# Starlight0798/gymRL

Measured on AMD Instinct MI355X. Metric: env-steps/sec at N envs/GPU (PPO LunarLander), 1/2/4/8 GPUs + %HBM roofline, higher is better.
Workload: dtype f32; 1 GPU; PPO LunarLander-v3, 4096 vectorised envs per MI355X (BASELINE.json configs[1]); envs_per_gpu=4096, rollout_len=2048, num_epochs=10, num_minibatches=32, minibatch=262144, model=ActorCritic 8-256-256-{256-4,256-1} tanh, 200,965 params, parallelism=single GPU

## Files before the change

### gymrl_amd/csrc/env_lunar_device.hpp

```cpp
#pragma once
#include "env_common.hpp"

namespace gymrl {
namespace lunar {


constexpr float kScale = 30.0f;
constexpr float kW = 600.0f / kScale;
constexpr float kH = 400.0f / kScale;
constexpr float kHelipadY = kH / 4.0f;
constexpr float kLegDown = 18.0f / kScale;
constexpr float kLegAway = 20.0f / kScale;
constexpr float kDt = 1.0f / 50.0f;
constexpr int kVelIters = 180, kPosIters = 60, kMaxSteps = 1000;
constexpr float kLinearSlopSqMax = 0x1.a36e30p-16f;
constexpr float kLinearSlop = 0.005f, kAngularSlop = 2.0f / 180.0f * 3.14159265359f;
constexpr float kPolyRadius = 2.0f * kLinearSlop;
constexpr float kMaxLinCorr = 0.2f, kMaxAngCorr = 8.0f / 180.0f * 3.14159265359f;
constexpr float kBaumgarte = 0.2f;
constexpr float kMaxTranslation = 2.0f, kMaxRotation = 0.5f * 3.14159265359f;
constexpr float kTimeToSleep = 0.5f, kLinSleepTol = 0.01f, kAngSleepTol = 2.0f / 180.0f * 3.14159265359f;
constexpr float kMotorTorque = 40.0f;

__device__ constexpr float kInvM[3] = {0.20761245674740486f, 14.0625f, 14.0625f};
// ... 294 lines not shown
    if (action == 2) {
      m_power = 1.0f;
      const float ox = tipx * (4.0f / kScale + 2.0f * disp0) + sidex * disp1;
      const float oy = -tipy * (4.0f / kScale + 2.0f * disp0) - sidey * disp1;
      const float ipx = posx + ox, ipy = posy + oy;
      const float Ix = -ox * 13.0f * m_power, Iy = -oy * 13.0f * m_power;
      B[0].vx += kInvM[0] * Ix; B[0].vy += kInvM[0] * Iy;
      B[0].w += kInvI[0] * cross2(ipx - B[0].cx, ipy - B[0].cy, Ix, Iy);
    }
    if (action == 1 || action == 3) {
      const float dir = (float)(action - 2);
      s_power = 1.0f;
      const float ox = tipx * disp0 + sidex * (3.0f * disp1 + dir * 12.0f / kScale);
      const float oy = -tipy * disp0 - sidey * (3.0f * disp1 + dir * 12.0f / kScale);
      const float ipx = posx + ox - tipx * 17.0f / kScale;
      const float ipy = posy + oy + tipy * 14.0f / kScale;
      const float Ix = -ox * 0.6f * s_power, Iy = -oy * 0.6f * s_power;
      B[0].vx += kInvM[0] * Ix; B[0].vy += kInvM[0] * Iy;
      B[0].w += kInvI[0] * cross2(ipx - B[0].cx, ipy - B[0].cy, Ix, Iy);
    }
  }

  uint32_t my_touch = 0u;
  bool my_contact = false;
  {
    const Body me = select_body(B, mb);
    float px, py, qs, qc;
    body_xf(me, lcy_, px, py, qs, qc);
    float minx = 3.4e38f, maxx = -3.4e38f, miny = 3.4e38f;
    if (is_hull) {
#pragma unroll
      for (int i = 0; i < 6; ++i) {
        const float x = (qc * kHullVx[i] - qs * kHullVy[i]) + px, y = (qs * kHullVx[i] + qc * kHullVy[i]) + py;
        minx = fminf(minx, x); maxx = fmaxf(maxx, x); miny = fminf(miny, y);
      }
    } else {
#pragma unroll
      for (int i = 0; i < 4; ++i) {
        const float x = (qc * kLegVx[i] - qs * kLegVy[i]) + px, y = (qs * kLegVx[i] + qc * kLegVy[i]) + py;
        minx = fminf(minx, x); maxx = fmaxf(maxx, x); miny = fminf(miny, y);
      }
    }
    int e_lo = (int)floorf((minx - 2.0f * kPolyRadius) * 0.5f);
    int e_hi = (int)floorf((maxx + 2.0f * kPolyRadius) * 0.5f);
    e_lo = e_lo < 0 ? 0 : e_lo;
    e_hi = e_hi > 9 ? 9 : e_hi;
    int ocount[2]; uint32_t okey[2][2]; float oni[2][2], oti[2][2];
#pragma unroll
    for (int os = 0; os < 2; ++os) {
      ocount[os] = (int)lds.mu(os, MF_COUNT);
#pragma unroll
      for (int q = 0; q < 2; ++q) {
        okey[os][q] = lds.mu(os, MF_P0 + 5 * q + P_KEY);
        oni[os][q] = lds.mf(os, MF_P0 + 5 * q + P_NI);
        oti[os][q] = lds.mf(os, MF_P0 + 5 * q + P_TI);
      }
    }
    const int old_e0 = W.edge0;
    W.edge0 = e_lo;
#pragma nounroll
    for (int s = 0; s < 2; ++s) {
      Manifold mf;
      mf.count = 0; mf.faceB = 0; mf.lnx = mf.lny = mf.lpx = mf.lpy = 0.0f;
      mf.p[0] = ContactPt{0.0f, 0.0f, 0u, 0.0f, 0.0f}; mf.p[1] = mf.p[0];
      const int e = e_lo + s;
      if (e <= e_hi && e >= 0 && e <= 9) {
        float y1 = W.ty[0], y2 = W.ty[1];
#pragma unroll
        for (int k = 0; k < 10; ++k) if (k == e) { y1 = W.ty[k]; y2 = W.ty[k + 1]; }
        const float x1 = 2.0f * (float)e, x2 = 2.0f * (float)(e + 1);
        if (miny - 2.0f * kPolyRadius <= fmaxf(y1, y2)) {
          const float ccx = is_hull ? me.cx : px, ccy = is_hull ? me.cy : py;
          if (is_hull) collide_edge_polygon<6>(mf, kHullVx, kHullVy, kHullNx, kHullNy, px, py, qs, qc, ccx, ccy, x1, y1, x2, y2);
          else collide_edge_polygon<4>(mf, kLegVx, kLegVy, kLegNx, kLegNy, px, py, qs, qc, ccx, ccy, x1, y1, x2, y2);
        }
#pragma unroll
        for (int k = 0; k < 2; ++k) {
          mf.p[k].ni = 0.0f; mf.p[k].ti = 0.0f;
          if (k < mf.count) {
            bool found = false;
#pragma unroll
            for (int os = 0; os < 2; ++os) {
              if (old_e0 + os == e) {
#pragma unroll
                for (int q = 0; q < 2; ++q)
                  if (!found && q < ocount[os] && okey[os][q] == mf.p[k].key) {
                    mf.p[k].ni = oni[os][q]; mf.p[k].ti = oti[os][q]; found = true;
                  }
              }
            }
          }
        }
        if (mf.count > 0) { my_touch |= 1u << e; my_contact = true; }
      }
      lds.mu(s, MF_COUNT) = (uint32_t)mf.count; lds.mu(s, MF_FACEB) = (uint32_t)mf.faceB;
      lds.mf(s, MF_LNX) = mf.lnx; lds.mf(s, MF_LNY) = mf.lny;
      lds.mf(s, MF_LPX) = mf.lpx; lds.mf(s, MF_LPY) = mf.lpy;
#pragma unroll
      for (int k = 0; k < 2; ++k) {
        lds.mf(s, MF_P0 + 5 * k + P_LPX) = mf.p[k].lpx; lds.mf(s, MF_P0 + 5 * k + P_LPY) = mf.p[k].lpy;
        lds.mu(s, MF_P0 + 5 * k + P_KEY) = mf.p[k].key;
        lds.mf(s, MF_P0 + 5 * k + P_NI) = mf.p[k].ni; lds.mf(s, MF_P0 + 5 * k + P_TI) = mf.p[k].ti;
      }
    }
  }
  const uint32_t touching_now = quad_bcast_u<0>(my_touch) | (quad_bcast_u<1>(my_touch) << 10) |
                                (quad_bcast_u<2>(my_touch) << 20);
  const bool any_contact = touching_now != 0u;
  {
    const uint32_t began = touching_now & ~W.touching, ended = W.touching & ~touching_now;
    if (began & 0x3FFu) W.flags |= 4u;
#pragma unroll
    for (int L = 0; L < 2; ++L) {
#pragma unroll
      for (int e = 0; e < 10; ++e) {
        const uint32_t bit = 1u << (10 * (L + 1) + e);
        if (began & bit) W.flags |= (1u << L);
        if (ended & bit) W.flags &= ~(1u << L);
      }
    }
    W.touching = touching_now;
  }

  LUNAR_PROF_MARK(pt1);
  LUNAR_PROF_ADD(lds, 0, pt0, pt1);
  const float h = kDt;
#pragma unroll
  for (int b = 0; b < 3; ++b) {
    const float Fx = b == 0 ? fx : 0.0f, Fy = b == 0 ? fy : 0.0f;
    B[b].vx += h * (0.0f + kInvM[b] * Fx);
    B[b].vy += h * (-10.0f + kInvM[b] * Fy);
  }

  int vcn[2] = {0, 0};
  float vcf[2][16], vim[2][4];
#pragma unroll
  for (int s = 0; s < 2; ++s) {
#pragma unroll
    for (int f = 0; f < 16; ++f) vcf[s][f] = 0.0f;
    vim[s][0] = vim[s][1] = vim[s][2] = vim[s][3] = 0.0f;
  }
  if (any_contact) {
    Body me = select_body(B, mb);
    if (my_contact) {
      float px, py, qs, qc;
      body_xf(me, lcy_, px, py, qs, qc);
#pragma unroll
      for (int s = 0; s < 2; ++s) {
        const int count = (int)lds.mu(s, MF_COUNT);
        int vcount = count;
        if (count > 0) {
          const bool faceB = lds.mu(s, MF_FACEB) != 0u;
          const float lnx = lds.mf(s, MF_LNX), lny = lds.mf(s, MF_LNY);
          const float lpx = lds.mf(s, MF_LPX), lpy = lds.mf(s, MF_LPY);
          float nx, ny, wpx[2], wpy[2];
          if (!faceB) {
            nx = lnx; ny = lny;
#pragma unroll
            for (int k = 0; k < 2; ++k) {
              const float qx = lds.mf(s, MF_P0 + 5 * k + P_LPX), qy = lds.mf(s, MF_P0 + 5 * k + P_LPY);
              const float clx = (qc * qx - qs * qy) + px, cly = (qs * qx + qc * qy) + py;
              const float d = kPolyRadius - dot2(clx - lpx, cly - lpy, nx, ny);
              const float cAx = clx + d * nx, cAy = cly + d * ny;
              const float cBx = clx - kPolyRadius * nx, cBy = cly - kPolyRadius * ny;
              wpx[k] = 0.5f * (cAx + cBx); wpy[k] = 0.5f * (cAy + cBy);
            }
          } else {
            nx = qc * lnx - qs * lny; ny = qs * lnx + qc * lny;
            const float ppx = (qc * lpx - qs * lpy) + px, ppy = (qs * lpx + qc * lpy) + py;
#pragma unroll
            for (int k = 0; k < 2; ++k) {
              const float clx = lds.mf(s, MF_P0 + 5 * k + P_LPX), cly = lds.mf(s, MF_P0 + 5 * k + P_LPY);
              const float d = kPolyRadius - dot2(clx - ppx, cly - ppy, nx, ny);
              const float cBx = clx + d * nx, cBy = cly + d * ny;
              const float cAx = clx - kPolyRadius * nx, cAy = cly - kPolyRadius * ny;
              wpx[k] = 0.5f * (cAx + cBx); wpy[k] = 0.5f * (cAy + cBy);
            }
            nx = -nx; ny = -ny;
          }
          const float tx = ny, ty = -nx;
          float rx[2], ry[2];
#pragma unroll
          for (int k = 0; k < 2; ++k) {
            rx[k] = wpx[k] - me.cx; ry[k] = wpy[k] - me.cy;
            const float rn = cross2(rx[k], ry[k], nx, ny);
            const float kn = mB_ + iB_ * rn * rn;
            vcf[s][VC_NM0 - 1 + k] = kn > 0.0f ? 1.0f / kn : 0.0f;
            const float rt = cross2(rx[k], ry[k], tx, ty);
            const float kt = mB_ + iB_ * rt * rt;
            vcf[s][VC_TM0 - 1 + k] = kt > 0.0f ? 1.0f / kt : 0.0f;
            vcf[s][VC_RX0 - 1 + 2 * k] = rx[k]; vcf[s][VC_RY0 - 1 + 2 * k] = ry[k];
          }
          vcf[s][VC_NX - 1] = nx; vcf[s][VC_NY - 1] = ny;
          if (count == 2) {
            const float rn1 = cross2(rx[0], ry[0], nx, ny), rn2 = cross2(rx[1], ry[1], nx, ny);
            const float k11 = mB_ + iB_ * rn1 * rn1, k22 = mB_ + iB_ * rn2 * rn2, k12 = mB_ + iB_ * rn1 * rn2;
            if (k11 * k11 < 1000.0f * (k11 * k22 - k12 * k12)) {
              float det = k11 * k22 - k12 * k12;
              if (det != 0.0f) det = 1.0f / det;
              vcf[s][VC_K11 - 1] = k11; vcf[s][VC_K12 - 1] = k12; vcf[s][VC_K22 - 1] = k22;
              vcf[s][VC_I11 - 1] = det * k22; vcf[s][VC_I12 - 1] = -det * k12; vcf[s][VC_I22 - 1] = det * k11;
            } else {
              vcount = 1;
            }
          }
          vim[s][0] = lds.mf(s, MF_P0 + P_NI); vim[s][1] = lds.mf(s, MF_P0 + P_TI);
          vim[s][2] = lds.mf(s, MF_P1 + P_NI); vim[s][3] = lds.mf(s, MF_P1 + P_TI);
#pragma unroll
          for (int k = 0; k < 2; ++k) {
            if (k < vcount) {
              const float ni = vim[s][2 * k], ti = vim[s][2 * k + 1];
              const float Px = ni * nx + ti * tx, Py = ni * ny + ti * ty;
              me.w += iB_ * cross2(rx[k], ry[k], Px, Py);
              me.vx += mB_ * Px; me.vy += mB_ * Py;
            }
          }
        }
        vcn[s] = vcount;
      }
    }
    quad_share_velocity(B, me);
  }

  float jrAx[2], jrAy[2], jrBx[2], jrBy[2];
  float K11[2], K12[2], K13[2], K22[2], K23[2], K33[2], mmass[2];
  {
    float qsA, qcA;
    det_sincosf(B[0].a, &qsA, &qcA);
#pragma unroll
    for (int jj = 0; jj < 2; ++jj) {
      const int L = 1 - jj;
      const int bi = L + 1;
      float qsB, qcB;
      det_sincosf(B[bi].a, &qsB, &qcB);
      const float lax = 0.0f - 0.0f, lay = 0.0f - kHullLcY;
      const float lbx = leg_sign(L) * kLegAway, lby = kLegDown;
      jrAx[L] = qcA * lax - qsA * lay; jrAy[L] = qsA * lax + qcA * lay;
      jrBx[L] = qcB * lbx - qsB * lby; jrBy[L] = qsB * lbx + qcB * lby;
      const float mA = kInvM[0], mB = kInvM[bi], iA = kInvI[0], iB = kInvI[bi];
      K11[L] = mA + mB + jrAy[L] * jrAy[L] * iA + jrBy[L] * jrBy[L] * iB;
      K12[L] = -jrAy[L] * jrAx[L] * iA - jrBy[L] * jrBx[L] * iB;
      K13[L] = -jrAy[L] * iA - jrBy[L] * iB;
      K22[L] = mA + mB + jrAx[L] * jrAx[L] * iA + jrBx[L] * jrBx[L] * iB;
      K23[L] = jrAx[L] * iA + jrBx[L] * iB;
      K33[L] = iA + iB;
      mmass[L] = 1.0f / (iA + iB);
      Joint& J = W.j[L];
      const float ang = B[bi].a - B[0].a;
      if (ang <= joint_lower(L)) { if (J.state != 1) J.iz = 0.0f; J.state = 1; }
      else if (ang >= joint_upper(L)) { if (J.state != 2) J.iz = 0.0f; J.state = 2; }
      else { J.state = 0; J.iz = 0.0f; }
      const float Px = J.ix, Py = J.iy;
      B[0].vx -= mA * Px; B[0].vy -= mA * Py;
      B[0].w -= iA * (cross2(jrAx[L], jrAy[L], Px, Py) + J.im + J.iz);
      B[bi].vx += mB * Px; B[bi].vy += mB * Py;
      B[bi].w += iB * (cross2(jrBx[L], jrBy[L], Px, Py) + J.im + J.iz);
    }
  }

  LUNAR_PROF_MARK(pt2);
  LUNAR_PROF_ADD(lds, 1, pt1, pt2);
  float jpAx[2], jpAy[2], jpBx[2], jpBy[2];
  float c1x[2], c1y[2], c1z[2], det3i[2], det2i[2], lim_sign[2];
  bool at_limit[2];
#pragma unroll
  for (int L = 0; L < 2; ++L) {
    const float a11 = K11[L], a12 = K12[L], a13 = K13[L], a22 = K22[L], a23 = K23[L], a33 = K33[L];
    c1x[L] = a22 * a33 - a23 * a23; c1y[L] = a23 * a13 - a12 * a33; c1z[L] = a12 * a23 - a22 * a13;
    float det = a11 * c1x[L] + a12 * c1y[L] + a13 * c1z[L];
    if (det != 0.0f) det = 1.0f / det;
    det3i[L] = det;
    float d2 = a11 * a22 - a12 * a12;
    if (d2 != 0.0f) d2 = 1.0f / d2;
    det2i[L] = d2;
    jpAx[L] = -jrAy[L]; jpAy[L] = jrAx[L]; jpBx[L] = -jrBy[L]; jpBy[L] = jrBx[L];
    at_limit[L] = W.j[L].state != 0;
    lim_sign[L] = W.j[L].state == 1 ? 1.0f : -1.0f;
  }
  const bool r0 = role == 0, r1 = role == 1, r2 = role == 2;
  auto lane3 = [&](float x, float y, float z) { return r0 ? x : (r1 ? y : (r2 ? z : 0.0f)); };
  float JPA[2], JPB[2], C1[2], P2[2], Q2[2], A2[2], P3[2], Q3[2], A3[2], A3C[2], D2[2], MBv[2], IBz[2];
#pragma unroll
  for (int L = 0; L < 2; ++L) {
    const float a11 = K11[L], a12 = K12[L], a13 = K13[L], a22 = K22[L], a23 = K23[L], a33 = K33[L];
    JPA[L] = lane3(jpAx[L], jpAy[L], 0.0f); JPB[L] = lane3(jpBx[L], jpBy[L], 0.0f);
    C1[L] = lane3(c1x[L], c1y[L], c1z[L]);
    P2[L] = lane3(a23, a33, a13); Q2[L] = lane3(a13, a23, a33); A2[L] = lane3(a13, a11, a12);
    P3[L] = lane3(a23, a12, a22); Q3[L] = lane3(a12, a22, a23); A3[L] = lane3(a12, a13, a11);
    A3C[L] = lane3(a13, a23, 0.0f); D2[L] = lane3(a22, a11, 0.0f);
    MBv[L] = lane3(kInvM[L + 1], kInvM[L + 1], kInvI[L + 1]); IBz[L] = r2 ? kInvI[L + 1] : 0.0f;
  }
  const float MAv = lane3(kInvM[0], kInvM[0], kInvI[0]), IAz = r2 ? kInvI[0] : 0.0f;
  float VA = lane3(B[0].vx, B[0].vy, B[0].w);
  float VB[2] = {lane3(B[1].vx, B[1].vy, B[1].w), lane3(B[2].vx, B[2].vy, B[2].w)};
  float JI[2] = {lane3(W.j[0].ix, W.j[0].iy, W.j[0].iz), lane3(W.j[1].ix, W.j[1].iy, W.j[1].iz)};
  float IM[2] = {W.j[0].im, W.j[1].im};
  const float maxImp = h * kMotorTorque;
#define SB __builtin_amdgcn_sched_barrier(0)
#define USEL(c, a, b) (__builtin_unpredictable(c) ? (a) : (b))
  float zb[2];
  zb[1] = quad_perm<0xAA>(JI[1]) * A3C[1];
  zb[0] = 0.0f;
  float lim_nan[2] = {at_limit[0] ? lim_sign[0] : __builtin_nanf(""), at_limit[1] ? lim_sign[1] : __builtin_nanf("")};
  asm volatile("" : "+v"(lim_nan[0]), "+v"(lim_nan[1]));
  auto joints = [&]() {
#pragma unroll
    for (int jj = 0; jj < 2; ++jj) {
      const int L = 1 - jj;
      const bool lim = at_limit[L];
      float t = VB[L] - VA; SB;
      t = t - 0.3f * leg_sign(L); SB;
      float imp = -mmass[L] * t; SB;
      float nw = IM[L] + imp; SB;
      nw = __builtin_amdgcn_fmed3f(nw, -maxImp, maxImp); SB;
      imp = nw - IM[L]; IM[L] = nw; SB;
      const float mb_ = IBz[L] * imp; SB;
      VB[L] = VB[L] + mb_; SB;
      const float ma_ = IAz * imp; SB;
      VA = VA - ma_; SB;
      const float xb = quad_perm<0xAA>(VB[L]) * JPB[L]; SB;
      float c = VB[L] + xb; SB;
      const float xa = quad_perm<0xAA>(VA) * JPA[L]; SB;
      c = c - VA; SB;
      c = c - xa; SB;
      const float u1 = c * C1[L]; SB;
      const float zc = zb[L] - c; SB;
      const float q2 = quad_perm<kRot1>(c) * Q2[L]; SB;
      const float q3 = quad_perm<kRot2>(c) * Q3[L]; SB;
      const float m2 = c * P2[L] - q2; SB;
      const float m3 = c * P3[L] - q3; SB;
      float s1 = quad_perm<kRot1>(u1) + u1; SB;
      const float u2 = A2[L] * m2; SB;
      const float u3 = A3[L] * m3; SB;
      s1 = quad_perm<kRot2>(u1) + s1; SB;
      const float rr = USEL(lim, zc, -c); SB;
      float s2 = quad_perm<kRot1>(u2) + u2; SB;
      float s3 = quad_perm<kRot1>(u3) + u3; SB;
      const float d2r = D2[L] * rr; SB;
      s2 = quad_perm<kRot2>(u2) + s2; SB;
      s3 = quad_perm<kRot2>(u3) + s3; SB;
      const float r2_ = quad_perm<kSwap01>(rr) * K12[L]; SB;
      float sel = USEL(r1, s2, s3); SB;
      sel = USEL(r0, s1, sel); SB;
      const float nsol = -(det3i[L] * sel); SB;
      const float newJ = JI[L] + nsol; SB;
      const float uu = d2r - r2_; SB;
      const float u = det2i[L] * uu; SB;
      const float rt = quad_perm<0xAA>(newJ) * lim_nan[L]; SB;
      const float altz = USEL(lim, -JI[L], 0.0f); SB;
      const float alt = USEL(r2, altz, u); SB;
      float ip;
      asm("v_cmp_nge_f32 vcc, %1, 0\n\tv_cndmask_b32_e32 %0, %2, %3, vcc" : "=v"(ip) : "v"(rt), "v"(nsol), "v"(alt) : "vcc"); SB;
      JI[L] = JI[L] + ip; SB;
      zb[1 - L] = quad_perm<0xAA>(JI[1 - L]) * A3C[1 - L]; SB;
      const float ay = quad_perm<0x55>(ip) * jrAx[L]; SB;
      const float ax = quad_perm<0x00>(ip) * jrAy[L]; SB;
      const float by = quad_perm<0x55>(ip) * jrBx[L]; SB;
      const float bx = quad_perm<0x00>(ip) * jrBy[L]; SB;
      const float crA = ay - ax; SB;
      const float crB = by - bx; SB;
      const float wA = crA + ip; SB;
      const float wB = crB + ip; SB;
      float tA = USEL(r2, wA, ip); SB;
      float tB = USEL(r2, wB, ip); SB;
      tA = MAv * tA; SB;
      tB = MBv[L] * tB; SB;
      VA = VA - tA; SB;
      VB[L] = VB[L] + tB; SB;
    }
  };
#undef SB
#undef USEL
  unsigned long long role_not1 = 0xDDDDDDDDDDDDDDDDull, role_not2 = 0xBBBBBBBBBBBBBBBBull, role_12 = 0x6666666666666666ull;
  asm volatile("" : "+s"(role_not1), "+s"(role_not2), "+s"(role_12));
#define QSEL3(d, s, R) "v_cndmask_b32_dpp " d ", " s ", " d ", vcc quad_perm:[" R "," R "," R "," R "] row_mask:0xf bank_mask:0xf bound_ctrl:1\n\t"
#define QMOV3(d, s, R) "v_mov_b32_dpp " d ", " s " quad_perm:[" R "," R "," R "," R "] row_mask:0xf bank_mask:0xf bound_ctrl:1\n\t"
  auto contacts = [&](auto two_, auto slot1_) {
    constexpr bool TWO = decltype(two_)::value, SLOT1 = decltype(slot1_)::value;
    const unsigned long long m_not1 = role_not1, m_not2 = role_not2, m_12 = role_12;
    if (any_contact) {
      Body me;
      me.cx = me.cy = me.a = 0.0f;
      asm(QMOV3("%0", "%5", "0") QMOV3("%1", "%5", "1") QMOV3("%2", "%5", "2")
          "s_mov_b64 vcc, %6\n\t"
          QSEL3("%0", "%4", "0") QSEL3("%1", "%4", "1") QSEL3("%2", "%4", "2")
          "s_mov_b64 vcc, %7\n\t"
          QSEL3("%0", "%3", "0") QSEL3("%1", "%3", "1") QSEL3("%2", "%3", "2")
          : "=&v"(me.vx), "=&v"(me.vy), "=&v"(me.w)
          : "v"(VA), "v"(VB[0]), "v"(VB[1]), "s"(m_not1), "s"(m_12)
          : "vcc");
#pragma unroll
      for (int s = 0; s < (SLOT1 ? 2 : 1); ++s) {
        const int vcount = vcn[s];
        if (vcount > 0) {
          const float nx = vcf[s][VC_NX - 1], ny = vcf[s][VC_NY - 1], tx = ny, ty = -nx;
          const float rx0 = vcf[s][VC_RX0 - 1], ry0 = vcf[s][VC_RY0 - 1], rx1 = vcf[s][VC_RX1 - 1], ry1 = vcf[s][VC_RY1 - 1];
          float ni0 = vim[s][0], ti0 = vim[s][1], ni1 = vim[s][2], ti1 = vim[s][3];
          {
            const float dvx = me.vx + (-me.w * ry0), dvy = me.vy + (me.w * rx0);
            const float vt = dot2(dvx, dvy, tx, ty);
            float lam = vcf[s][VC_TM0 - 1] * (-vt);
            const float maxF = fr_ * ni0;
            const float nw = clampf(ti0 + lam, -maxF, maxF);
            lam = nw - ti0; ti0 = nw;
            const float Px = lam * tx, Py = lam * ty;
            me.vx += mB_ * Px; me.vy += mB_ * Py;
            me.w += iB_ * cross2(rx0, ry0, Px, Py);
          }
          if (TWO && vcount == 2) {
            const float dvx = me.vx + (-me.w * ry1), dvy = me.vy + (me.w * rx1);
            const float vt = dot2(dvx, dvy, tx, ty);
            float lam = vcf[s][VC_TM1 - 1] * (-vt);
            const float maxF = fr_ * ni1;
            const float nw = clampf(ti1 + lam, -maxF, maxF);
            lam = nw - ti1; ti1 = nw;
            const float Px = lam * tx, Py = lam * ty;
            me.vx += mB_ * Px; me.vy += mB_ * Py;
            me.w += iB_ * cross2(rx1, ry1, Px, Py);
          }
          if (!TWO || vcount == 1) {
            const float dvx = me.vx + (-me.w * ry0), dvy = me.vy + (me.w * rx0);
            const float vn = dot2(dvx, dvy, nx, ny);
            float lam = -vcf[s][VC_NM0 - 1] * vn;
            const float nw = fmaxf(ni0 + lam, 0.0f);
            lam = nw - ni0; ni0 = nw;
            const float Px = lam * nx, Py = lam * ny;
            me.vx += mB_ * Px; me.vy += mB_ * Py;
            me.w += iB_ * cross2(rx0, ry0, Px, Py);
          } else {
            const float k11 = vcf[s][VC_K11 - 1], k12 = vcf[s][VC_K12 - 1], k22 = vcf[s][VC_K22 - 1];
            const float a1 = ni0, a2 = ni1;
            const float dv1x = me.vx + (-me.w * ry0), dv1y = me.vy + (me.w * rx0);
            const float dv2x = me.vx + (-me.w * ry1), dv2y = me.vy + (me.w * rx1);
            float vn1 = dot2(dv1x, dv1y, nx, ny), vn2 = dot2(dv2x, dv2y, nx, ny);
            const float b1 = vn1 - (k11 * a1 + k12 * a2);
            const float b2 = vn2 - (k12 * a1 + k22 * a2);
            float x1 = -(vcf[s][VC_I11 - 1] * b1 + vcf[s][VC_I12 - 1] * b2);
            float x2 = -(vcf[s][VC_I12 - 1] * b1 + vcf[s][VC_I22 - 1] * b2);
            bool ok = (x1 >= 0.0f && x2 >= 0.0f);
            if (!ok) {
              x1 = -vcf[s][VC_NM0 - 1] * b1; x2 = 0.0f;
              vn2 = k12 * x1 + b2;
              ok = (x1 >= 0.0f && vn2 >= 0.0f);
            }
            if (!ok) {
              x1 = 0.0f; x2 = -vcf[s][VC_NM1 - 1] * b2;
              vn1 = k12 * x2 + b1;
              ok = (x2 >= 0.0f && vn1 >= 0.0f);
            }
            if (!ok) {
              x1 = 0.0f; x2 = 0.0f;
              ok = (b1 >= 0.0f && b2 >= 0.0f);
            }
            if (ok) {
              const float d1 = x1 - a1, d2 = x2 - a2;
              const float P1x = d1 * nx, P1y = d1 * ny, P2x = d2 * nx, P2y = d2 * ny;
              me.vx += mB_ * (P1x + P2x); me.vy += mB_ * (P1y + P2y);
              me.w += iB_ * (cross2(rx0, ry0, P1x, P1y) + cross2(rx1, ry1, P2x, P2y));
              ni0 = x1; ni1 = x2;
            }
          }
          vim[s][0] = ni0; vim[s][1] = ti0;
          if (TWO && vcount == 2) { vim[s][2] = ni1; vim[s][3] = ti1; }
        }
      }
      asm("s_mov_b64 vcc, %6\n\t"
          QMOV3("%0", "%3", "0") QMOV3("%1", "%3", "1") QMOV3("%2", "%3", "2")
          QSEL3("%0", "%4", "0") QSEL3("%1", "%4", "1") QSEL3("%2", "%4", "2")
          "s_mov_b64 vcc, %7\n\t"
          QSEL3("%0", "%5", "0") QSEL3("%1", "%5", "1") QSEL3("%2", "%5", "2")
          : "=&v"(VA), "=&v"(VB[0]), "=&v"(VB[1])
          : "v"(me.vx), "v"(me.vy), "v"(me.w), "s"(m_not1), "s"(m_not2)
          : "vcc");
    }
  };
#undef QSEL3
#undef QMOV3
  const bool wave_two = __builtin_amdgcn_ballot_w64(vcn[0] == 2 || vcn[1] == 2) != 0ull || lds.general_sweep;
  const bool wave_slot1 = __builtin_amdgcn_ballot_w64(vcn[1] > 0) != 0ull;
  if (__builtin_amdgcn_ballot_w64(any_contact) == 0ull) {
#pragma nounroll
    for (int it = 0; it < kVelIters; ++it) joints();
  } else if (wave_two) {
#pragma nounroll
    for (int it = 0; it < kVelIters; ++it) { joints(); contacts(SweepFlag<true>{}, SweepFlag<true>{}); }
  } else if (wave_slot1) {
#pragma nounroll
    for (int it = 0; it < kVelIters; ++it) { joints(); contacts(SweepFlag<false>{}, SweepFlag<true>{}); }
  } else {
#pragma nounroll
    for (int it = 0; it < kVelIters; ++it) { joints(); contacts(SweepFlag<false>{}, SweepFlag<false>{}); }
  }
  B[0].vx = quad_bcast<0>(VA); B[0].vy = quad_bcast<1>(VA); B[0].w = quad_bcast<2>(VA);
#pragma unroll
  for (int L = 0; L < 2; ++L) {
    B[L + 1].vx = quad_bcast<0>(VB[L]); B[L + 1].vy = quad_bcast<1>(VB[L]); B[L + 1].w = quad_bcast<2>(VB[L]);
    W.j[L].ix = quad_bcast<0>(JI[L]); W.j[L].iy = quad_bcast<1>(JI[L]); W.j[L].iz = quad_bcast<2>(JI[L]);
    W.j[L].im = quad_bcast<2>(IM[L]);
  }
  LUNAR_PROF_MARK(pt3);
  LUNAR_PROF_ADD(lds, 2, pt2, pt3);
#ifdef GYMRL_LUNAR_PROF
  const bool wave_contact = __builtin_amdgcn_ballot_w64(any_contact) != 0ull;
  LUNAR_PROF_ADD(lds, wave_contact ? 6 : 7, pt2, pt3);
#endif
  if (my_contact) {
#pragma unroll
    for (int s = 0; s < 2; ++s) {
      if (vcn[s] > 0) {
        lds.mf(s, MF_P0 + P_NI) = vim[s][0]; lds.mf(s, MF_P0 + P_TI) = vim[s][1];
        if (vcn[s] == 2) { lds.mf(s, MF_P1 + P_NI) = vim[s][2]; lds.mf(s, MF_P1 + P_TI) = vim[s][3]; }
      }
    }
  }

#pragma unroll
  for (int b = 0; b < 3; ++b) {
    float tx = h * B[b].vx, ty = h * B[b].vy;
    if (dot2(tx, ty, tx, ty) > kMaxTranslation * kMaxTranslation) {
      const float ratio = kMaxTranslation / sqrtf(dot2(tx, ty, tx, ty));
      B[b].vx *= ratio; B[b].vy *= ratio;
    }
    const float rot = h * B[b].w;
    if (rot * rot > kMaxRotation * kMaxRotation) {
      const float ratio = kMaxRotation / fabsf(rot);
      B[b].w *= ratio;
    }
    B[b].cx += h * B[b].vx; B[b].cy += h * B[b].vy; B[b].a += h * B[b].w;
  }

  LUNAR_PROF_MARK(pt4);
  LUNAR_PROF_ADD(lds, 3, pt3, pt4);
#ifdef GYMRL_LUNAR_PROF
  int prof_pos_iters = 0;
#endif
  bool position_solved = false;
  float plim_value[2], plim_slop[2], plim_lo[2], plim_hi[2];
#pragma unroll
  for (int L = 0; L < 2; ++L) {
    const bool lower = W.j[L].state == 1;
    plim_value[L] = lower ? joint_lower(L) : joint_upper(L);
    plim_slop[L] = lower ? kAngularSlop : -kAngularSlop;
    plim_lo[L] = lower ? -kMaxAngCorr : 0.0f;
    plim_hi[L] = lower ? 0.0f : kMaxAngCorr;
  }
  int pcnt[2] = {0, 0};
  bool pfaceB[2] = {false, false};
  float plnx[2], plny[2], plpx[2], plpy[2], pqx[2][2], pqy[2][2];
#pragma unroll
  for (int s = 0; s < 2; ++s) {
    plnx[s] = plny[s] = plpx[s] = plpy[s] = 0.0f;
    pqx[s][0] = pqx[s][1] = pqy[s][0] = pqy[s][1] = 0.0f;
    if (my_contact) {
      pcnt[s] = (int)lds.mu(s, MF_COUNT);
      pfaceB[s] = lds.mu(s, MF_FACEB) != 0u;
      plnx[s] = lds.mf(s, MF_LNX); plny[s] = lds.mf(s, MF_LNY);
      plpx[s] = lds.mf(s, MF_LPX); plpy[s] = lds.mf(s, MF_LPY);
#pragma unroll
      for (int k = 0; k < 2; ++k) {
        pqx[s][k] = lds.mf(s, MF_P0 + 5 * k + P_LPX); pqy[s][k] = lds.mf(s, MF_P0 + 5 * k + P_LPY);
      }
    }
  }
#pragma nounroll
  for (int it = 0; it < kPosIters; ++it) {
    float min_sep = 0.0f;
    if (any_contact) {
      Body me = select_body(B, mb);
      float my_min = 0.0f;
#pragma unroll
      for (int s = 0; s < 2; ++s) {
        const int cnt = pcnt[s];
        if (cnt > 0) {
          const bool faceB = pfaceB[s];
          const float lnx = plnx[s], lny = plny[s], lpx = plpx[s], lpy = plpy[s];
#pragma unroll
          for (int k = 0; k < 2; ++k) {
            if (k < cnt) {
              const float qx = pqx[s][k], qy = pqy[s][k];
              float px, py, qs, qc;
              body_xf(me, lcy_, px, py, qs, qc);
              float nx, ny, ptx, pty, sep;
              if (!faceB) {
                nx = lnx; ny = lny;
                const float clx = (qc * qx - qs * qy) + px, cly = (qs * qx + qc * qy) + py;
                sep = dot2(clx - lpx, cly - lpy, nx, ny) - kPolyRadius - kPolyRadius;
                ptx = clx; pty = cly;
              } else {
                nx = qc * lnx - qs * lny; ny = qs * lnx + qc * lny;
                const float ppx = (qc * lpx - qs * lpy) + px, ppy = (qs * lpx + qc * lpy) + py;
                sep = dot2(qx - ppx, qy - ppy, nx, ny) - kPolyRadius - kPolyRadius;
                ptx = qx; pty = qy;
                nx = -nx; ny = -ny;
              }
              const float rx = ptx - me.cx, ry = pty - me.cy;
              my_min = fminf(my_min, sep);
              const float C = clampf(kBaumgarte * (sep + kLinearSlop), -kMaxLinCorr, 0.0f);
              const float rn = cross2(rx, ry, nx, ny);
              const float K = mB_ + iB_ * rn * rn;
              const float imp = K > 0.0f ? -C / K : 0.0f;
              const float Px = imp * nx, Py = imp * ny;
              me.cx += mB_ * Px; me.cy += mB_ * Py;
              me.a += iB_ * cross2(rx, ry, Px, Py);
            }
          }
        }
      }
      quad_share_position(B, me);
      min_sep = fminf(fminf(quad_bcast<0>(my_min), quad_bcast<1>(my_min)), quad_bcast<2>(my_min));
    }
    const bool contacts_ok = min_sep >= -3.0f * kLinearSlop;
    bool joints_ok = true;
#pragma unroll
    for (int jj = 0; jj < 2; ++jj) {
      const int L = 1 - jj;
      const int bi = L + 1;
      const float mA = kInvM[0], mB = kInvM[bi], iA = kInvI[0], iB = kInvI[bi];
      const bool lim = at_limit[L];
      const float Cang = (B[bi].a - B[0].a) - plim_value[L];
      const float angErr = lim ? -(lim_sign[L] * Cang) : 0.0f;
      const float Cc = clampf(Cang + plim_slop[L], plim_lo[L], plim_hi[L]);
      const float limImp = lim ? -mmass[L] * Cc : 0.0f;
      B[0].a -= iA * limImp; B[bi].a += iB * limImp;
      float qsA, qcA, qsB, qcB;
      {
        float sn, cs;
        det_sincosf((role & 1) ? B[bi].a : B[0].a, &sn, &cs);
        qsA = quad_bcast<0>(sn); qcA = quad_bcast<0>(cs);
        qsB = quad_bcast<1>(sn); qcB = quad_bcast<1>(cs);
      }
      const float lax = 0.0f, lay = 0.0f - kHullLcY;
      const float lbx = leg_sign(L) * kLegAway, lby = kLegDown;
      const float rAx = qcA * lax - qsA * lay, rAy = qsA * lax + qcA * lay;
      const float rBx = qcB * lbx - qsB * lby, rBy = qsB * lbx + qcB * lby;
      const float Cx = B[bi].cx + rBx - B[0].cx - rAx, Cy = B[bi].cy + rBy - B[0].cy - rAy;
      const float posErr2 = Cx * Cx + Cy * Cy;
      const float k11 = mA + mB + iA * rAy * rAy + iB * rBy * rBy;
      const float k12 = -iA * rAx * rAy - iB * rBx * rBy;
      const float k22 = mA + mB + iA * rAx * rAx + iB * rBx * rBx;
      float det = k11 * k22 - k12 * k12;
      if (det != 0.0f) det = 1.0f / det;
      const float impx = -(det * (k22 * Cx - k12 * Cy)), impy = -(det * (k11 * Cy - k12 * Cx));
      B[0].cx -= mA * impx; B[0].cy -= mA * impy;
      B[0].a -= iA * cross2(rAx, rAy, impx, impy);
      B[bi].cx += mB * impx; B[bi].cy += mB * impy;
      B[bi].a += iB * cross2(rBx, rBy, impx, impy);
      joints_ok = joints_ok && (posErr2 <= kLinearSlopSqMax) && (angErr <= kAngularSlop);
#ifdef GYMRL_LUNAR_PROF
      if (it == 10 && lds.prof && role == 0) {
        if (!(posErr2 <= kLinearSlopSqMax)) atomicAdd(&lds.prof[14], 1ull);
        if (!(angErr <= kAngularSlop)) atomicAdd(&lds.prof[15], 1ull);
      }
#endif
    }
#ifdef GYMRL_LUNAR_PROF
    if (it == 10 && lds.prof && role == 0) {
      if (!contacts_ok) atomicAdd(&lds.prof[13], 1ull);
      atomicAdd(&lds.prof[5], 1ull);
    }
#endif
    if (contacts_ok && joints_ok) { position_solved = true; break; }
#ifdef GYMRL_LUNAR_PROF
    ++prof_pos_iters;
#endif
  }
#ifdef GYMRL_LUNAR_PROF
  {
    int wmax = prof_pos_iters + (position_solved ? 1 : 0), mine = wmax;
    for (int off = 32; off > 0; off >>= 1) wmax = max(wmax, __shfl_xor(wmax, off, 64));
    if (lds.prof && (threadIdx.x & 63) == 0) { lds.prof[11] += (unsigned long long)wmax; lds.prof[12] += (unsigned long long)mine; }
    if (lds.envp && role == 0) {
      lds.envp[0] += any_contact ? 1ull : 0ull;
      lds.envp[lds.envn] += (unsigned long long)mine;
      lds.envp[2 * (size_t)lds.envn] += wave_contact ? 1ull : 0ull;
    }
  }
#endif

  LUNAR_PROF_MARK(pt5);
  LUNAR_PROF_ADD(lds, 4, pt4, pt5);
  float min_sleep = 3.4e38f;
#pragma unroll
  for (int b = 0; b < 3; ++b) {
    if (B[b].w * B[b].w > kAngSleepTol * kAngSleepTol ||
        dot2(B[b].vx, B[b].vy, B[b].vx, B[b].vy) > kLinSleepTol * kLinSleepTol) {
      W.sleep[b] = 0.0f; min_sleep = 0.0f;
    } else {
      W.sleep[b] += h;
      min_sleep = fminf(min_sleep, W.sleep[b]);
    }
  }
  if (min_sleep >= kTimeToSleep && position_solved) W.flags |= 16u;
}

__device__ __forceinline__ void lander_obs(const World& W, float (&o)[8]) {
  float sn, cs;
  det_sincosf(W.b[0].a, &sn, &cs);
  const float posx = W.b[0].cx - (cs * 0.0f - sn * kHullLcY);
  const float posy = W.b[0].cy - (sn * 0.0f + cs * kHullLcY);
  o[0] = (posx - kW / 2.0f) / (kW / 2.0f);
  o[1] = (posy - (kHelipadY + kLegDown)) / (kH / 2.0f);
  o[2] = W.b[0].vx * (kW / 2.0f) / 50.0f;
  o[3] = W.b[0].vy * (kH / 2.0f) / 50.0f;
  o[4] = W.b[0].a;
  o[5] = 20.0f * W.b[0].w / 50.0f;
  o[6] = (W.flags & 1u) ? 1.0f : 0.0f;
  o[7] = (W.flags & 2u) ? 1.0f : 0.0f;
}

__device__ __forceinline__ float shaping_of(const float (&o)[8]) {
  return -100.0f * sqrtf(o[0] * o[0] + o[1] * o[1]) - 100.0f * sqrtf(o[2] * o[2] + o[3] * o[3]) -
         100.0f * fabsf(o[4]) + 10.0f * o[6] + 10.0f * o[7];
}

__device__ __forceinline__ void env_step_once(World& W, const Lds& lds, int role, int action, uint64_t seed,
                                              uint64_t env, uint32_t episode, uint32_t step_idx, float fx,
                                              float fy, float (&o)[8], float& reward, bool& terminated) {
  const u32x4 r = philox4x32(seed, (uint32_t)env, (uint32_t)(env >> 32), episode, RNG_ENV_STEP | step_idx);
  const float d0 = (-1.0f + 2.0f * u01f(r.x)) / kScale, d1 = (-1.0f + 2.0f * u01f(r.y)) / kScale;
  float mp, sp;
  world_step(W, lds, role, action, d0, d1, fx, fy, mp, sp);
  lander_obs(W, o);
  const float shaping = shaping_of(o);
  reward = 0.0f;
  if (W.flags & 8u) reward = shaping - W.prev_shaping;
  W.prev_shaping = shaping; W.flags |= 8u;
  reward -= mp * 0.30f;
  reward -= sp * 0.03f;
  terminated = false;
  if ((W.flags & 4u) || fabsf(o[0]) >= 1.0f) { terminated = true; reward = -100.0f; }
  if (W.flags & 16u) { terminated = true; reward = 100.0f; }
}

__device__ __forceinline__ void init_episode(World& W, const Lds& lds, uint64_t seed, uint64_t env,
                                             uint32_t episode, float& fx, float& fy) {
  float hgt[12];
#pragma unroll
  for (int blk = 0; blk < 3; ++blk) {
    const u32x4 r = philox4x32(seed, (uint32_t)env, (uint32_t)(env >> 32), episode, RNG_ENV_RESET | (uint32_t)blk);
    hgt[4 * blk + 0] = (kH / 2.0f) * u01f(r.x); hgt[4 * blk + 1] = (kH / 2.0f) * u01f(r.y);
    hgt[4 * blk + 2] = (kH / 2.0f) * u01f(r.z); hgt[4 * blk + 3] = (kH / 2.0f) * u01f(r.w);
  }
#pragma unroll
  for (int i = 3; i <= 7; ++i) hgt[i] = kHelipadY;
#pragma unroll
  for (int i = 0; i < 11; ++i) {
    const float prev = hgt[i == 0 ? 11 : i - 1];
    W.ty[i] = 0.33f * (prev + hgt[i] + hgt[i + 1]);
  }
  const u32x4 rf = philox4x32(seed, (uint32_t)env, (uint32_t)(env >> 32), episode, RNG_ENV_RESET | 3u);
  fx = -1000.0f + 2000.0f * u01f(rf.x); fy = -1000.0f + 2000.0f * u01f(rf.y);
  W.b[0] = Body{kW / 2.0f, kH + kHullLcY, 0.0f, 0.0f, 0.0f, 0.0f};
#pragma unroll
  for (int L = 0; L < 2; ++L) {
    const float i = leg_sign(L);
    W.b[L + 1] = Body{kW / 2.0f - i * kLegAway, kH, i * 0.05f, 0.0f, 0.0f, 0.0f};
    W.j[L] = Joint{0.0f, 0.0f, 0.0f, 0.0f, 0};
  }
#pragma unroll
  for (int b = 0; b < 3; ++b) W.sleep[b] = 0.0f;
  W.edge0 = 0;
#pragma nounroll
  for (int k = 0; k < 2 * kMfWords; ++k) lds.w[k * kEnvBlock] = 0u;
  W.touching = 0u; W.flags = 0u; W.prev_shaping = 0.0f;
}

constexpr int kWorldWords = 18 + 3 + 10 + 3 * 2 * kMfWords + 3 + 1 + 11 + 1 + 1;
constexpr int kWMf = 31, kWEdge0 = 31 + 96, kWTail = 31 + 96 + 3;

constexpr uint32_t kNoSpare = 0xFFFFFFFFu;

struct LunarState {
  uint32_t* words;
  EpisodeFields ep;
  uint32_t* spare_words;
  float* spare_obs;
  uint32_t* spare_episode;
  size_t bytes;
  __host__ __device__ LunarState(void* buf, int n) {
    Carver c(buf, n);
    words = c.take<uint32_t>(kWorldWords);
    ep.ep_ret = c.take<double>(); ep.ep_len = c.take<int32_t>(); ep.episode = c.take<uint32_t>();
    spare_words = c.take<uint32_t>(kWorldWords);
    spare_obs = c.take<float>(8);
    spare_episode = c.take<uint32_t>();
    bytes = c.off;
  }
};

struct WordIO {
  uint32_t* base; int n; int i; int k; bool wr;
  __device__ __forceinline__ void f(float& x, bool store) {
    if (store) { if (wr) base[(size_t)k * n + i] = __float_as_uint(x); } else x = __uint_as_float(base[(size_t)k * n + i]);
    ++k;
  }
// ... 206 lines not shown
```

Before: 7.312 million env-steps/s.

## Specialize velocity sweeps for all-at-limit joints and leg-only contact waves

Adds compile-time variants of the Box2D velocity-iteration loop. When every lane in a wave has both leg joints at their angular limit, the joint solver skips the lower-limit fallback computation unless a wave ballot shows some lane's accumulated impulse went negative. When no hull contacts exist in the wave, the contact solver skips gathering and scattering the hull body's velocity. This trims instructions in the 180-iteration inner loop, at the cost of more kernel code paths (instruction cache pressure) and an added per-iteration ballot branch.

New measurement: 7.322 million env-steps/s (median of 2 runs). Within noise of the previous version (+0.1%).

```diff
diff --git a/gymrl_amd/csrc/env_lunar_device.hpp b/gymrl_amd/csrc/env_lunar_device.hpp
--- a/gymrl_amd/csrc/env_lunar_device.hpp
+++ b/gymrl_amd/csrc/env_lunar_device.hpp
@@ -620,12 +620,14 @@
   zb[1] = quad_perm<0xAA>(JI[1]) * A3C[1];
   zb[0] = 0.0f;
   float lim_nan[2] = {at_limit[0] ? lim_sign[0] : __builtin_nanf(""), at_limit[1] ? lim_sign[1] : __builtin_nanf("")};
-  asm volatile("" : "+v"(lim_nan[0]), "+v"(lim_nan[1]));
-  auto joints = [&]() {
+  float lim_l2[2] = {r2 ? lim_sign[0] : 0.0f, r2 ? lim_sign[1] : 0.0f};
+  asm volatile("" : "+v"(lim_nan[0]), "+v"(lim_nan[1]), "+v"(lim_l2[0]), "+v"(lim_l2[1]));
+  auto joints = [&](auto all_lim_) {
+    constexpr bool ALL_LIM = decltype(all_lim_)::value;
 #pragma unroll
     for (int jj = 0; jj < 2; ++jj) {
       const int L = 1 - jj;
-      const bool lim = at_limit[L];
+      const bool lim = ALL_LIM || at_limit[L];
       float t = VB[L] - VA; SB;
       t = t - 0.3f * leg_sign(L); SB;
       float imp = -mmass[L] * t; SB;
@@ -642,7 +644,8 @@
       c = c - VA; SB;
       c = c - xa; SB;
       const float u1 = c * C1[L]; SB;
-      const float zc = zb[L] - c; SB;
+      float zc = 0.0f;
+      if constexpr (!ALL_LIM) { zc = zb[L] - c; SB; }
       const float q2 = quad_perm<kRot1>(c) * Q2[L]; SB;
       const float q3 = quad_perm<kRot2>(c) * Q3[L]; SB;
       const float m2 = c * P2[L] - q2; SB;
@@ -651,40 +654,69 @@
       const float u2 = A2[L] * m2; SB;
       const float u3 = A3[L] * m3; SB;
       s1 = quad_perm<kRot2>(u1) + s1; SB;
-      const float rr = USEL(lim, zc, -c); SB;
+      float rr = 0.0f;
+      if constexpr (!ALL_LIM) { rr = USEL(lim, zc, -c); SB; }
       float s2 = quad_perm<kRot1>(u2) + u2; SB;
       float s3 = quad_perm<kRot1>(u3) + u3; SB;
-      const float d2r = D2[L] * rr; SB;
+      float d2r = 0.0f;
+      if constexpr (!ALL_LIM) { d2r = D2[L] * rr; SB; }
       s2 = quad_perm<kRot2>(u2) + s2; SB;
       s3 = quad_perm<kRot2>(u3) + s3; SB;
-      const float r2_ = quad_perm<kSwap01>(rr) * K12[L]; SB;
+      float r2_ = 0.0f;
+      if constexpr (!ALL_LIM) { r2_ = quad_perm<kSwap01>(rr) * K12[L]; SB; }
       float sel = USEL(r1, s2, s3); SB;
       sel = USEL(r0, s1, sel); SB;
       const float nsol = -(det3i[L] * sel); SB;
       const float newJ = JI[L] + nsol; SB;
-      const float uu = d2r - r2_; SB;
-      const float u = det2i[L] * uu; SB;
-      const float rt = quad_perm<0xAA>(newJ) * lim_nan[L]; SB;
-      const float altz = USEL(lim, -JI[L], 0.0f); SB;
-      const float alt = USEL(r2, altz, u); SB;
-      float ip;
-      asm("v_cmp_nge_f32 vcc, %1, 0\n\tv_cndmask_b32_e32 %0, %2, %3, vcc" : "=v"(ip) : "v"(rt), "v"(nsol), "v"(alt) : "vcc"); SB;
-      JI[L] = JI[L] + ip; SB;
-      zb[1 - L] = quad_perm<0xAA>(JI[1 - L]) * A3C[1 - L]; SB;
-      const float ay = quad_perm<0x55>(ip) * jrAx[L]; SB;
-      const float ax = quad_perm<0x00>(ip) * jrAy[L]; SB;
-      const float by = quad_perm<0x55>(ip) * jrBx[L]; SB;
-      const float bx = quad_perm<0x00>(ip) * jrBy[L]; SB;
-      const float crA = ay - ax; SB;
-      const float crB = by - bx; SB;
-      const float wA = crA + ip; SB;
-      const float wB = crB + ip; SB;
-      float tA = USEL(r2, wA, ip); SB;
-      float tB = USEL(r2, wB, ip); SB;
-      tA = MAv * tA; SB;
-      tB = MBv[L] * tB; SB;
-      VA = VA - tA; SB;
-      VB[L] = VB[L] + tB; SB;
+      auto apply = [&](float ip) {
+        const float ay = quad_perm<0x55>(ip) * jrAx[L]; SB;
+        const float ax = quad_perm<0x00>(ip) * jrAy[L]; SB;
+        const float by = quad_perm<0x55>(ip) * jrBx[L]; SB;
+        const float bx = quad_perm<0x00>(ip) * jrBy[L]; SB;
+        const float crA = ay - ax; SB;
+        const float crB = by - bx; SB;
+        const float wA = crA + ip; SB;
+        const float wB = crB + ip; SB;
+        float tA = USEL(r2, wA, ip); SB;
+        float tB = USEL(r2, wB, ip); SB;
+        tA = MAv * tA; SB;
+        tB = MBv[L] * tB; SB;
+        VA = VA - tA; SB;
+        VB[L] = VB[L] + tB; SB;
+      };
+      if constexpr (!ALL_LIM) {
+        const float uu = d2r - r2_; SB;
+        const float u = det2i[L] * uu; SB;
+        const float rt = quad_perm<0xAA>(newJ) * lim_nan[L]; SB;
+        const float altz = USEL(lim, -JI[L], 0.0f); SB;
+        const float alt = USEL(r2, altz, u); SB;
+        float ip;
+        asm("v_cmp_nge_f32 vcc, %1, 0\n\tv_cndmask_b32_e32 %0, %2, %3, vcc" : "=v"(ip) : "v"(rt), "v"(nsol), "v"(alt) : "vcc"); SB;
+        JI[L] = JI[L] + ip; SB;
+        zb[1 - L] = quad_perm<0xAA>(JI[1 - L]) * A3C[1 - L]; SB;
+        apply(ip);
+      } else {
+        const float rt2 = newJ * lim_l2[L]; SB;
+        float ip;
+        if (__builtin_expect(__builtin_amdgcn_ballot_w64(!(rt2 >= 0.0f)) != 0ull, 0)) {
+          const float zbL = quad_perm<0xAA>(JI[L]) * A3C[L]; SB;
+          const float zcL = zbL - c; SB;
+          const float d2rL = D2[L] * zcL; SB;
+          const float r2L = quad_perm<kSwap01>(zcL) * K12[L]; SB;
+          const float uu = d2rL - r2L; SB;
+          const float u = det2i[L] * uu; SB;
+          const float rt = quad_perm<0xAA>(newJ) * lim_sign[L]; SB;
+          const float altz = -JI[L]; SB;
+          const float alt = USEL(r2, altz, u); SB;
+          asm("v_cmp_nge_f32 vcc, %1, 0\n\tv_cndmask_b32_e32 %0, %2, %3, vcc" : "=v"(ip) : "v"(rt), "v"(nsol), "v"(alt) : "vcc"); SB;
+          JI[L] = JI[L] + ip; SB;
+        } else {
+          ip = nsol;
+          JI[L] = newJ;
+        }
+        apply(ip);
+        asm volatile("" : "+v"(VB[L]));
+      }
     }
   };
 #undef SB
@@ -693,20 +725,29 @@
   asm volatile("" : "+s"(role_not1), "+s"(role_not2), "+s"(role_12));
 #define QSEL3(d, s, R) "v_cndmask_b32_dpp " d ", " s ", " d ", vcc quad_perm:[" R "," R "," R "," R "] row_mask:0xf bank_mask:0xf bound_ctrl:1\n\t"
 #define QMOV3(d, s, R) "v_mov_b32_dpp " d ", " s " quad_perm:[" R "," R "," R "," R "] row_mask:0xf bank_mask:0xf bound_ctrl:1\n\t"
-  auto contacts = [&](auto two_, auto slot1_) {
-    constexpr bool TWO = decltype(two_)::value, SLOT1 = decltype(slot1_)::value;
+  auto contacts = [&](auto two_, auto slot1_, auto hull_) {
+    constexpr bool TWO = decltype(two_)::value, SLOT1 = decltype(slot1_)::value, HULL = decltype(hull_)::value;
     const unsigned long long m_not1 = role_not1, m_not2 = role_not2, m_12 = role_12;
     if (any_contact) {
       Body me;
       me.cx = me.cy = me.a = 0.0f;
-      asm(QMOV3("%0", "%5", "0") QMOV3("%1", "%5", "1") QMOV3("%2", "%5", "2")
-          "s_mov_b64 vcc, %6\n\t"
-          QSEL3("%0", "%4", "0") QSEL3("%1", "%4", "1") QSEL3("%2", "%4", "2")
-          "s_mov_b64 vcc, %7\n\t"
-          QSEL3("%0", "%3", "0") QSEL3("%1", "%3", "1") QSEL3("%2", "%3", "2")
-          : "=&v"(me.vx), "=&v"(me.vy), "=&v"(me.w)
-          : "v"(VA), "v"(VB[0]), "v"(VB[1]), "s"(m_not1), "s"(m_12)
-          : "vcc");
+      if constexpr (HULL) {
+        asm(QMOV3("%0", "%5", "0") QMOV3("%1", "%5", "1") QMOV3("%2", "%5", "2")
+            "s_mov_b64 vcc, %6\n\t"
+            QSEL3("%0", "%4", "0") QSEL3("%1", "%4", "1") QSEL3("%2", "%4", "2")
+            "s_mov_b64 vcc, %7\n\t"
+            QSEL3("%0", "%3", "0") QSEL3("%1", "%3", "1") QSEL3("%2", "%3", "2")
+            : "=&v"(me.vx), "=&v"(me.vy), "=&v"(me.w)
+            : "v"(VA), "v"(VB[0]), "v"(VB[1]), "s"(m_not1), "s"(m_12)
+            : "vcc");
+      } else {
+        asm(QMOV3("%0", "%4", "0") QMOV3("%1", "%4", "1") QMOV3("%2", "%4", "2")
+            "s_mov_b64 vcc, %5\n\t"
+            QSEL3("%0", "%3", "0") QSEL3("%1", "%3", "1") QSEL3("%2", "%3", "2")
+            : "=&v"(me.vx), "=&v"(me.vy), "=&v"(me.w)
+            : "v"(VB[0]), "v"(VB[1]), "s"(m_not1)
+            : "vcc");
+      }
 #pragma unroll
       for (int s = 0; s < (SLOT1 ? 2 : 1); ++s) {
         const int vcount = vcn[s];
@@ -782,33 +823,51 @@
           if (TWO && vcount == 2) { vim[s][2] = ni1; vim[s][3] = ti1; }
         }
       }
-      asm("s_mov_b64 vcc, %6\n\t"
-          QMOV3("%0", "%3", "0") QMOV3("%1", "%3", "1") QMOV3("%2", "%3", "2")
-          QSEL3("%0", "%4", "0") QSEL3("%1", "%4", "1") QSEL3("%2", "%4", "2")
-          "s_mov_b64 vcc, %7\n\t"
-          QSEL3("%0", "%5", "0") QSEL3("%1", "%5", "1") QSEL3("%2", "%5", "2")
-          : "=&v"(VA), "=&v"(VB[0]), "=&v"(VB[1])
-          : "v"(me.vx), "v"(me.vy), "v"(me.w), "s"(m_not1), "s"(m_not2)
-          : "vcc");
+      if constexpr (HULL) {
+        asm("s_mov_b64 vcc, %6\n\t"
+            QMOV3("%0", "%3", "0") QMOV3("%1", "%3", "1") QMOV3("%2", "%3", "2")
+            QSEL3("%0", "%4", "0") QSEL3("%1", "%4", "1") QSEL3("%2", "%4", "2")
+            "s_mov_b64 vcc, %7\n\t"
+            QSEL3("%0", "%5", "0") QSEL3("%1", "%5", "1") QSEL3("%2", "%5", "2")
+            : "=&v"(VA), "=&v"(VB[0]), "=&v"(VB[1])
+            : "v"(me.vx), "v"(me.vy), "v"(me.w), "s"(m_not1), "s"(m_not2)
+            : "vcc");
+      } else {
+        asm("s_mov_b64 vcc, %5\n\t"
+            QMOV3("%0", "%2", "1") QMOV3("%1", "%2", "2")
+            QSEL3("%0", "%3", "1") QSEL3("%1", "%3", "2")
+            "s_mov_b64 vcc, %6\n\t"
+            QSEL3("%0", "%4", "1") QSEL3("%1", "%4", "2")
+            : "=&v"(VB[0]), "=&v"(VB[1])
+            : "v"(me.vx), "v"(me.vy), "v"(me.w), "s"(m_not1), "s"(m_not2)
+            : "vcc");
+      }
     }
   };
 #undef QSEL3
 #undef QMOV3
   const bool wave_two = __builtin_amdgcn_ballot_w64(vcn[0] == 2 || vcn[1] == 2) != 0ull || lds.general_sweep;
   const bool wave_slot1 = __builtin_amdgcn_ballot_w64(vcn[1] > 0) != 0ull;
-  if (__builtin_amdgcn_ballot_w64(any_contact) == 0ull) {
+  const bool wave_hull = __builtin_amdgcn_ballot_w64(is_hull && (vcn[0] > 0 || vcn[1] > 0)) != 0ull;
+  const bool wave_lim = __builtin_amdgcn_ballot_w64(!(at_limit[0] && at_limit[1])) == 0ull && !lds.general_sweep;
+  auto sweeps = [&](auto lim_, auto contact_, auto two_, auto slot1_, auto hull_) {
 #pragma nounroll
-    for (int it = 0; it < kVelIters; ++it) joints();
-  } else if (wave_two) {
-#pragma nounroll
-    for (int it = 0; it < kVelIters; ++it) { joints(); contacts(SweepFlag<true>{}, SweepFlag<true>{}); }
-  } else if (wave_slot1) {
-#pragma nounroll
-    for (int it = 0; it < kVelIters; ++it) { joints(); contacts(SweepFlag<false>{}, SweepFlag<true>{}); }
-  } else {
-#pragma nounroll
-    for (int it = 0; it < kVelIters; ++it) { joints(); contacts(SweepFlag<false>{}, SweepFlag<false>{}); }
-  }
+    for (int it = 0; it < kVelIters; ++it) {
+      joints(lim_);
+      if constexpr (decltype(contact_)::value) contacts(two_, slot1_, hull_);
+    }
+  };
+  auto sweeps_lim = [&](auto contact_, auto two_, auto slot1_, auto hull_) {
+    if (wave_lim) sweeps(SweepFlag<true>{}, contact_, two_, slot1_, hull_);
+    else sweeps(SweepFlag<false>{}, contact_, two_, slot1_, hull_);
+  };
+  constexpr SweepFlag<true> yes{};
+  constexpr SweepFlag<false> no{};
+  if (__builtin_amdgcn_ballot_w64(any_contact) == 0ull) sweeps_lim(no, no, no, no);
+  else if (wave_two) sweeps_lim(yes, yes, yes, yes);
+  else if (wave_hull) sweeps_lim(yes, no, yes, yes);
+  else if (wave_slot1) sweeps_lim(yes, no, yes, no);
+  else sweeps_lim(yes, no, no, no);
   B[0].vx = quad_bcast<0>(VA); B[0].vy = quad_bcast<1>(VA); B[0].w = quad_bcast<2>(VA);
 #pragma unroll
   for (int L = 0; L < 2; ++L) {
```
